# Ledicia/Molecular-Dynamics-Simulation---Lennard-Jones-monoatomic-fluid

Hardware: AMD Instinct MI355X
Metric: md_steps_per_sec_n262144_fp64 (higher is better)
Workload: dtype f64

## Files before the change

molecular-dynamics-simulation---lennard-jones-monoatomic-fluid_amd/csrc/ljmd_common.cpp:

```cpp
#include "ljmd_common.h"
#include "ljmd_internal.h"

#include <algorithm>
#include <cstdio>
#include <cstring>
#include <limits>

namespace ljmdh {

using namespace ljmdk;

thread_local std::string g_last_error = "";

int failv(std::string *handle_err, int code, const char *fmt, va_list ap)
{
    char buf[512];
    vsnprintf(buf, sizeof buf, fmt, ap);
    g_last_error = buf;
    if (handle_err) *handle_err = buf;
    return code;
}

int check_sim_params(const char *who, int n, double box_length, double dt, double rc)
{
// ... 51 lines not shown
        if (v && *v) return std::atoi(v);
        return std::nullopt;
    };
    Knobs k;
    k.sort = flag("LJMD_SORT", k.sort);
    k.force_generic = flag("LJMD_FORCE_GENERIC", k.force_generic);
    k.force_collectives = flag("LJMD_FORCE_COLLECTIVES", k.force_collectives);
    k.fuse = flag("LJMD_FUSE", k.fuse);
    k.fuse_tail = flag("LJMD_FUSE_TAIL", k.fuse_tail);
    k.fuse_defer_record = flag("LJMD_FUSE_DEFER_RECORD", k.fuse_defer_record);
    k.xcd_remap = std::max(0, env_int("LJMD_N3_XCD_REMAP", k.xcd_remap));
    k.inject_failure_at_step = env_int("LJMD_INJECT_FAILURE_AT_STEP", k.inject_failure_at_step);
    k.exchange_alltoall = is("LJMD_FORCE_EXCHANGE", "alltoall");
    k.resort_every = opt_int("LJMD_RESORT_EVERY");
    k.n3_row_tiles = env_int("LJMD_N3_ROW_TILES", k.n3_row_tiles);
    k.n3_wg_waves = env_int("LJMD_N3_WG_WAVES", k.n3_wg_waves);
    k.slab_budget_gb = std::max(1, env_int("LJMD_SLAB_BUDGET_GB", k.slab_budget_gb));
    k.n3_both_ties = flag("LJMD_N3_BOTH_TIES", k.n3_both_ties);
    k.n3_min_n = env_int("LJMD_N3_MIN_N", k.n3_min_n);
    k.n3 = flag("LJMD_N3", k.n3);
    k.n3_target_waves = opt_int("LJMD_N3_TARGET_WAVES");
    k.n3_clusters = flag("LJMD_N3_CLUSTERS", k.n3_clusters);
    k.n3_pertile = flag("LJMD_N3_PERTILE", k.n3_pertile);
    k.fp32_far_stream = flag("LJMD_FP32_FAR_STREAM", k.fp32_far_stream);
    k.fp32_vfar = flag("LJMD_FP32_VFAR", k.fp32_vfar);
    {
        const char *rs = std::getenv("LJMD_FP32_SPLIT");
        if (rs && *rs) k.fp32_split = std::max(0.0, std::atof(rs));
    }
    k.overlap_exchange = flag("LJMD_OVERLAP_EXCHANGE", k.overlap_exchange);
    k.migrate_blocks = is("LJMD_MIGRATE_DEAL", "blocks");
    {
        const char *xm = std::getenv("LJMD_MULTI_EXCHANGE");
        k.multi_exchange = xm ? xm : "";
    }
    k.multi_migrate_every = std::max(0, env_int("LJMD_MULTI_MIGRATE_EVERY", k.multi_migrate_every));
    k.multi_threads = flag("LJMD_MULTI_THREADS", k.multi_threads);
    k.batch_group_streams = !is("LJMD_BATCH_GROUP_STREAMS", "0");
    return k;
}

void scalars_from_sums(double s12, double s6, double kx, double ky, double kz, double te, double td, double tdd,
                       double *epot, double *ekin, double *d_epot, double *dd_epot)
{
    if (epot) *epot = 4.0 * (s12 - s6) + te;
    if (d_epot) *d_epot = 24.0 * (-2.0 * s12 + s6) + td;
// ... 67 lines not shown
```

molecular-dynamics-simulation---lennard-jones-monoatomic-fluid_amd/csrc/ljmd_common.h:

```cpp
#ifndef LJMD_COMMON_H
#define LJMD_COMMON_H

#include "ljmd.h"

#include <hip/hip_runtime.h>

#include <cstdarg>
#include <cstddef>
#include <cstdint>
#include <cstdlib>
#include <optional>
#include <string>

namespace ljmdh {

extern thread_local std::string g_last_error;

constexpr double kPi = 3.1415926535897932384626433832795;

int failv(std::string *handle_err, int code, const char *fmt, va_list ap);

inline int fail(std::nullptr_t, int code, const char *fmt, ...)
{
    va_list ap;
// ... 49 lines not shown
void scalars_from_exact_sums(const uint64_t (&ordered)[5][3], double te, double td, double tdd, bool have_e, bool have_k,
                             double *epot, double *ekin, double *d_epot, double *dd_epot);

struct Knobs {
    bool sort = true;
    bool force_generic = false;
    bool force_collectives = false;
    bool fuse = true;
    bool fuse_tail = true;
    bool fuse_defer_record = true;
    int xcd_remap = 4;
    int inject_failure_at_step = -1;
    bool exchange_alltoall = false;
    std::optional<int> resort_every;
    int n3_row_tiles = 0;
    int n3_wg_waves = 0;
    int slab_budget_gb = 64;
    bool n3_both_ties = true;
    int n3_min_n = 4096;
    bool n3 = true;
    std::optional<int> n3_target_waves;
    bool n3_clusters = true;
    bool n3_pertile = true;
    bool fp32_far_stream = true;
    bool fp32_vfar = true;
    double fp32_split = 5.0;
    bool overlap_exchange = true;
    bool migrate_blocks = false;
    std::string multi_exchange;
    int multi_migrate_every = 2000;
    bool multi_threads = true;
    bool batch_group_streams = true;
};
Knobs read_knobs();

}
#endif
```

molecular-dynamics-simulation---lennard-jones-monoatomic-fluid_amd/csrc/ljmd_engine.cpp:

```cpp
#include "ljmd_engine.h"

namespace ljmdh {

bool fast_path_ok(const ljmd_t *h) { return h->plan.rc_allows_fast && h->positions_compact && !h->knobs.force_generic; }

double *wg_part_now(ljmd_t *h) { return h->d_wg_part + (h->plan.fuse_tail ? (size_t)h->fold_parity * h->wg_part_stride : 0); }

PairArgs pair_args(ljmd_t *h, bool fast)
{
    PairArgs a;
    a.pos = h->d_pos;
    a.slab = h->d_slab;
    a.wg_part = wg_part_now(h);
    a.mask = h->d_mask;
    a.bbox = h->d_bbox;
    a.inline_mask = (fast && h->plan.fuse_tail && !h->plan.use_n3) ? 1 : 0;
    a.rc2_skin = h->rc2 * (1.0 + 1e-10);
    a.n = h->n;
    a.S = h->plan.S;
    a.P = h->plan.P;
    a.G = h->G;
    a.rank = h->rank;
    a.TB = h->plan.TB;
    a.T = h->plan.T;
// ... 36 lines not shown
    a.pos = h->d_pos_tc;
    a.mask = h->d_mask;
    a.bbox = h->d_bbox;
    a.desc = h->d_desc;
    a.desc2 = h->d_desc2;
    a.slab_i = h->d_slab;
    a.slab_j = h->d_slab_j;
    a.flag_j = h->d_flag_j;
    a.wg_part = wg_part_now(h);
    a.S = h->plan.S;
    a.P = h->plan.P;
    a.G = h->G;
    a.rank = h->rank;
    a.TB = h->plan.TB;
    a.T = h->plan.T;
    a.W = h->plan.W;
    a.NG = h->plan.NG;
    a.NGo = h->plan.NGo;
    a.Dmax = h->plan.Dmax;
    a.CS = h->plan.CS;
    a.by_group = h->plan.j_by_group;
    a.dchunk = h->plan.dchunk;
    a.uchunk = h->plan.uchunk;
    a.xcd_remap = 0;
    a.inline_class = (h->plan.fuse_tail && h->plan.rt <= 2 && h->plan.wg_waves == 1) ? 1 : 0;
    a.both_ties = h->plan.both_ties ? 1 : 0;
    a.rc2_skin = h->rc2 * (1.0 + 1e-10);
    a.energy = h->want_energy ? 1 : 0;
    a.RT = h->plan.rt;
    a.L = h->L;
    a.invL = h->invL;
    a.rc2 = h->rc2;
    return a;
}

IntegrateArgs integrate_args(ljmd_t *h)
{
    IntegrateArgs a;
    a.r = own_block(h);
    a.ru = h->d_ru;
    a.v = h->d_v;
    a.a = h->d_a;
    a.fsum = needs_force_exchange(h) ? h->d_frecv : h->d_fpart;
    a.bbox = nullptr;
    a.pos_tc = nullptr;
    a.RT = std::max(1, h->plan.rt);
// ... 6 lines not shown
    a.dt = h->dt;
    a.dt_half = h->dt_half;
    a.dt_sq_half = h->dt_sq_half;
    return a;
}

ReduceArgs reduce_args(ljmd_t *h, int nslab, bool n3)
{
    ReduceArgs a;
    a.slab = h->d_slab;
    a.slab_j = n3 ? h->d_slab_j : nullptr;
    a.flag_j = n3 ? h->d_flag_j : nullptr;
    a.slab_j2 = (n3 && h->mode == LJMD_PRECISION_FP32_FORCE) ? reinterpret_cast<const float *>(h->d_slab_j2) : nullptr;
    a.flag_j2 = (n3 && h->mode == LJMD_PRECISION_FP32_FORCE) ? h->d_flag_j2 : nullptr;
    a.fpart = h->d_fpart;
    a.nslab = nslab;
    a.P = h->plan.P;
    a.G = h->G;
    a.rank = h->rank;
    a.TB = h->plan.TB;
    a.CS = h->plan.CS;
    a.CS2 = h->plan.CS2;
    a.RT = h->plan.rt;
    return a;
}

FinalizeArgs finalize_args(ljmd_t *h, int n_wg, bool with_ke, double pair_scale)
{
    FinalizeArgs a;
    a.pair_scale = pair_scale;
    a.wg_part = wg_part_now(h);
    a.ke_part = h->d_ke_part;
    a.ke_tile = nullptr;
    a.ring = h->d_ring;
    a.ring_pos = h->d_ring_pos;
    a.n_wg = n_wg;
    a.n_ke = with_ke ? h->plan.n_ke : 0;
    a.ring_cap = kRingCap;
    return a;
}

EventSet *next_events(ljmd_t *h)
{
    if (!h->profiling || h->ev_used >= (size_t)kMaxProfiledLaunches) return nullptr;
    if (h->ev_used == h->ev_pool.size()) {
        EventSet q;
// ... 84 lines not shown
            LJMD_HIP(h, launch_tile_mask(ga, h->stream));
        }
        h->boxes_valid = false;
        if (q) LJMD_HIP(h, hipEventRecord(q->e[2], h->stream));
        FixedArgs fa;
        fa.pos = h->d_pos;
        fa.mask = h->d_mask;
        fa.fslab = h->d_fslab;
        fa.fflag = h->d_fflag;
        fa.walk_all = fast ? 0 : 1;
        fa.S = h->plan.S; fa.P = h->plan.P; fa.G = h->G; fa.rank = h->rank; fa.TB = h->plan.TB; fa.T = h->plan.T; fa.W = h->plan.W;
        fa.chunk = h->plan.chunk_t;
        fa.energy = h->want_energy ? 1 : 0;
        fa.L = h->L; fa.invL = h->invL; fa.rc2 = h->rc2;
        LJMD_HIP(h, launch_pair_fixed(fa, dim3(h->plan.TB / kWavesPerBlock, h->plan.nslab_t), h->stream));
        if (q) LJMD_HIP(h, hipEventRecord(q->e[3], h->stream));
        h->pending_energy = h->want_energy;
        h->reduce_deferred = false;
        h->forces_pending = true;
        return LJMD_OK;
    }
    int nslab, n_wg;
    bool n3 = false;
    if (fast) {
        GeometryArgs ga = geometry_args(h);
        if (!h->plan.use_n3) ga.mask_far = nullptr;
        if (!h->boxes_valid) LJMD_HIP(h, launch_tile_boxes(ga, h->stream));
        h->boxes_valid = false;
        if (h->plan.fuse_tail)
            ;
        else if (h->plan.use_n3)
            LJMD_HIP(h, launch_tile_class(ga, h->invL, h->rc2, h->plan.S, h->plan.NGo, h->d_desc,
                                          h->mode == LJMD_PRECISION_FP32_FORCE ? h->d_desc_far : nullptr, h->d_desc2, h->stream));
        else
            LJMD_HIP(h, launch_tile_mask(ga, h->stream));
        if (q) LJMD_HIP(h, hipEventRecord(q->e[2], h->stream));
        if (h->plan.use_n3) {
            const dim3 grid((h->plan.NGo + h->plan.wg_waves - 1) / h->plan.wg_waves, h->plan.nslab_n);
            N3Args na = n3_args(h);
            na.xcd_remap = (h->knobs.xcd_remap > 0 && (int)grid.x >= kXcdMinGroups && grid.x % (8 * h->knobs.xcd_remap) == 0) ? h->knobs.xcd_remap : 0;
            const bool far_beside = h->mode == LJMD_PRECISION_FP32_FORCE && h->far_stream != nullptr;
            if (far_beside) {
                LJMD_HIP(h, hipEventRecord(h->ev_far_go, h->stream));
                LJMD_HIP(h, hipStreamWaitEvent(h->far_stream, h->ev_far_go, 0));
            } else {
                LJMD_HIP(h, launch_pair_n3(na, grid, h->plan.wg_waves, h->stream));
            }
            nslab = h->plan.nslab_n;
            n_wg = grid.x * grid.y * h->plan.wg_waves;
            n3 = true;
            if (h->mode == LJMD_PRECISION_FP32_FORCE) {
                const dim3 fgrid(h->plan.NGo, h->plan.nslab_n);
                N3Args fa = n3_args(h);
                fa.mask = h->d_mask_far;
                fa.slab_i = h->d_slab + (size_t)h->plan.nslab_n * 3 * h->plan.P;
                fa.slab_j = h->d_slab_j2;
                fa.flag_j = h->d_flag_j2;
                fa.desc = h->d_desc_far;
                fa.CS = h->plan.CS2;
                fa.by_group = h->G > 1 ? 1 : 0;
                fa.xcd_remap = (h->knobs.xcd_remap > 0 && (int)fgrid.x >= kXcdMinGroups && fgrid.x % (8 * h->knobs.xcd_remap) == 0) ? h->knobs.xcd_remap : 0;
                fa.wg_part = h->d_wg_part + 2 * (size_t)n_wg;
                LJMD_HIP(h, launch_pair_n3_f32(fa, fgrid, far_beside ? h->far_stream : h->stream));
                if (far_beside) {
                    LJMD_HIP(h, hipEventRecord(h->ev_far_done, h->far_stream));
// ... 4 lines not shown
                n_wg += fgrid.x * fgrid.y;
            }
        } else {
            const dim3 grid(h->plan.TB / kWavesPerBlock, h->plan.nslab_t);
            LJMD_HIP(h, launch_pair_tiles(pair_args(h, true), grid, h->stream));
            nslab = h->plan.nslab_t;
            n_wg = grid.x * grid.y;
        }
    } else {
        if (h->plan.use_n3 && h->G > 1)
            return fail(h, LJMD_ERR_STATE,
                        "multi-rank Newton-3 run needs wrapped positions and rc <= (1-1e-9) L/2 (set LJMD_N3=0)");
        if (q) LJMD_HIP(h, hipEventRecord(q->e[2], h->stream));
        const dim3 grid(h->plan.P / kBlock, h->plan.nslab_g);
        LJMD_HIP(h, launch_pair_rows_generic(pair_args(h, false), grid, h->stream));
        nslab = h->plan.nslab_g;
        n_wg = grid.x * grid.y;
    }
    if (q) LJMD_HIP(h, hipEventRecord(q->e[3], h->stream));
    h->reduce_deferred = fast && h->plan.fuse_tail && h->kick_hint >= 0 && n_wg <= kDirectFoldMax && !needs_force_exchange(h);
    if (h->reduce_deferred) {
        h->deferred_nslab = nslab;
        h->deferred_n3 = n3;
    } else {
        LJMD_HIP(h, launch_reduce_forces(reduce_args(h, nslab, n3), needs_force_exchange(h), h->stream));
    }
    h->forces_pending = true;
    h->pending_n_wg = n_wg;
    h->pending_scale = n3 ? 1.0 : 0.5;
    return LJMD_OK;
}

int enqueue_kick(ljmd_t *h, bool kick, EventSet *q)
{
    if (reproducible(h)) {
        FixedTailArgs ta;
        ta.fslab = h->d_fslab;
        ta.fflag = h->d_fflag;
        ta.nslab = h->plan.nslab_t;
        ta.P = h->plan.P;
        ta.TB = h->plan.TB;
        ta.a = h->d_a;
        ta.v = h->d_v;
        ta.dt_half = h->dt_half;
        ta.blk = h->d_fblk;
        LJMD_HIP(h, launch_fixed_tail(ta, kick, h->pending_energy, false, h->stream));
// ... 196 lines not shown
```

molecular-dynamics-simulation---lennard-jones-monoatomic-fluid_amd/csrc/ljmd_engine.h:

```cpp
#ifndef LJMD_ENGINE_H
#define LJMD_ENGINE_H

#include "ljmd_common.h"

#include <rccl/rccl.h>

#include <algorithm>
#include <cmath>
#include <cstdio>
#include <cstring>
#include <limits>
#include <mutex>
#include <vector>

#include "ljmd_internal.h"
#include "ljmd_rdf.h"
#include "ljmd_tcf.h"

using namespace ljmdk;

namespace ljmdh {

constexpr unsigned kRingCap = 4096;
constexpr int kTargetWorkgroups = 2048;
constexpr int kXcdMinGroups = 256;
constexpr int kMixedMinN = 16384;
constexpr long kN3ItemsFor4 = 6000;
constexpr long kN3ItemsFor2 = 1000;
constexpr long kN3LargeItems = 131072;
constexpr int kN3MidTargetItems = 32768;
constexpr int kBothTiesMaxGroups = 128;
constexpr int kFuseTailMaxRowTiles = 2;
constexpr int kFuseTailMaxN = 20000;
constexpr int kMaxProfiledLaunches = 4096;
constexpr int kEventsPerLaunch = 9;

struct EventSet {
    hipEvent_t e[kEventsPerLaunch];
    bool has_pos_x = false, has_force_x = false;
};

struct LaunchPlan {
    int S = 0, P = 0;
    int TB = 0, T = 0, W = 0;
    bool rc_allows_fast = false;
    bool sort_enabled = true;
    int resort_every = 20;
    std::vector<int> kd_level_nseg;
    std::vector<size_t> kd_level_off;
    std::vector<int> kd_offsets;
    int nslab_g = 1, chunk_g = 0;
    int nslab_t = 1, chunk_t = 0;
    bool use_n3 = false;
    int wg_waves = 1;
    bool both_ties = false;
    int uchunk = 0;
    int CS = 0, CS2 = 0, j_by_group = 0;
    int NG = 0, NGo = 0, Dmax = 0, nslab_n = 1, dchunk = 0;
    int rt = kRowTiles;
    bool fuse_tail = false;
    int nslab_max = 1, n_wg_max = 0;
    int n_ke = 0;
};

int plan_engine(const SimParams &sim, int n, int n_ranks, int precision_mode, const Knobs &k, LaunchPlan *out);

}

struct ljmd_multi;

using namespace ljmdh;

struct ljmd : ljmdh::SimParams {
    ljmd_multi *multi = nullptr;
    bool poisoned = false;
    int inject_failure_at = -1;
    int n = 0, rank = 0, G = 1, device = 0, mode = 0;
    ljmdh::Knobs knobs;
    ljmdh::LaunchPlan plan;
    bool tail_on = true;
    bool positions_compact = false;
    bool have_state = false, have_accel = false;
    int steps_since_sort = 0;
// ... 28 lines not shown
    unsigned *d_ring_pos = nullptr;
    double *d_bbox = nullptr;
    uint64_t *d_mask = nullptr;
    double *d_pos_tc = nullptr;
    unsigned *d_desc = nullptr;
    unsigned *d_desc_far = nullptr;
    float *d_desc2 = nullptr;
    int *d_idx = nullptr, *d_idx2 = nullptr, *d_perm = nullptr, *d_perm2 = nullptr;
    double *d_tmp3 = nullptr;
    void *d_cub = nullptr;
    size_t cub_bytes = 0;
    std::vector<int> kd_axis;
    int *d_kd_offsets = nullptr;
    unsigned long long *d_kd_keys = nullptr, *d_kd_keys2 = nullptr;

    unsigned ring_consumed = 0;
    unsigned ring_issued = 0;
    bool fold_pending = false;
    ljmdk::FinalizeArgs pending_fold{};
    int fold_parity = 0;
    size_t wg_part_stride = 0;
    double *d_slab_j = nullptr;
    unsigned char *d_flag_j = nullptr;
    uint64_t *d_mask_far = nullptr;
    double *d_slab_j2 = nullptr;
    unsigned char *d_flag_j2 = nullptr;
    double *d_fpart = nullptr, *d_frecv = nullptr;
    double *d_fall = nullptr;
    bool forces_pending = false;
    bool external_force_exchange = false;
    int pending_n_wg = 0;
    double pending_scale = 0.5;

    double *h_stage = nullptr;
    double *h_ring = nullptr;
    std::vector<int> h_perm;
    bool perm_dirty = false;

    hipStream_t far_stream = nullptr;
    hipEvent_t ev_far_go = nullptr, ev_far_done = nullptr;
    hipStream_t copy_stream = nullptr;
    hipEvent_t ev_snap_ready = nullptr, ev_snap_done = nullptr;
    double *d_snap = nullptr, *h_snap = nullptr;
    int *d_snap_perm = nullptr, *h_snap_perm = nullptr;
    bool snap_in_flight = false;
    bool snap_ready = false;
// ... 72 lines not shown
```

molecular-dynamics-simulation---lennard-jones-monoatomic-fluid_amd/csrc/ljmd_internal.h:

```cpp
#ifndef LJMD_INTERNAL_H
#define LJMD_INTERNAL_H

#include <hip/hip_runtime.h>
#include <stdint.h>

namespace ljmdk {

constexpr int kBlock = 256;
constexpr int kWavesPerBlock = kBlock / 64;
constexpr int kTile = 64;
#ifndef LJMD_ROW_TILES
#define LJMD_ROW_TILES 4
#endif
constexpr int kRowTiles = LJMD_ROW_TILES;
constexpr unsigned kAllRows = (1u << kRowTiles) - 1u;
constexpr int kSlotAlign = (kRowTiles * 64 > 256) ? kRowTiles * 64 : 256;
constexpr int kPartialStride = 8;
constexpr int kFoldBlocks = 128;
constexpr int kDirectFoldMax = 20480;
constexpr int kBoxStride = 8;

struct PairArgs {
    const double *pos;
    double *slab;
// ... 9 lines not shown
    int rank;
    int TB;
    int T;
    int W;
    int chunk;
    double L, invL, rc2;
};

struct N3Args {
    const double *pos;
    const uint64_t *mask;
    const double *bbox;
    const unsigned *desc;
    const float *desc2;
    double *slab_i;
    double *slab_j;
    unsigned char *flag_j;
    double *wg_part;
    int S, P, G, rank, TB, T, W;
    int NG, NGo, Dmax;
    int CS, by_group;
    int RT;
    int dchunk;
    int uchunk;
    int energy;
    int xcd_remap;
    int inline_class;
    int both_ties;
    double L, invL, rc2;
    double rc2_skin;
};

struct IntegrateArgs {
    double *r;
    double *ru, *v, *a;
    const double *fsum;
    double *ke_part;
    int rows;
    int P;
    double L, invL, dt, dt_half, dt_sq_half;
    double *bbox;
    double *pos_tc;
    int RT;
    unsigned *ticket;
};

struct ReduceArgs {
    const double *slab;
    const double *slab_j;
    const unsigned char *flag_j;
    const float *slab_j2;
    const unsigned char *flag_j2;
    double *fpart;
    int nslab, P, G, rank, TB;
    int CS, CS2;
    int RT;
};

struct FinalizeArgs {
    const double *wg_part;
    const double *ke_part;
    const double *ke_tile;
    double *ring;
    unsigned *ring_pos;
    int n_wg, n_ke;
    unsigned ring_cap;
    double pair_scale;
};

struct GeometryArgs {
    const double *pos;
    double *bbox;
    double *pos_tc;
    uint64_t *mask;
    uint64_t *mask_far;
    int P, G, rank, TB, T, W;
    int RT;
    double L, invL, rc2_skin;
    double rsplit2;
// ... 97 lines not shown
    return neg ? -r : r;
}

struct RdfArgs {
    const double *x, *y, *z;
    unsigned long long *hist;
    int n, nbins, chunk;
    double L, rmax, dr;
    double invL, inv_dr;
};

struct TimeOriginArgs {
    const double *x, *y, *z;
    double *term;
    int n_snap, n, max_lag, origin_stride;
};

hipError_t launch_pair_rows_generic(const PairArgs &a, dim3 grid, hipStream_t s);
hipError_t launch_pair_tiles(const PairArgs &a, dim3 grid, hipStream_t s);
hipError_t launch_pair_n3(const N3Args &a, dim3 grid, int wg_waves, hipStream_t s);
hipError_t launch_pair_n3_f32(const N3Args &a, dim3 grid, hipStream_t s);
hipError_t launch_drift_kick(const IntegrateArgs &a, int phase , hipStream_t s);
hipError_t launch_reduce_forces(const ReduceArgs &a, bool all_blocks, hipStream_t s);
hipError_t launch_kick(const IntegrateArgs &a, bool kick, hipStream_t s);
hipError_t launch_kick_finalize(const IntegrateArgs &a, const FinalizeArgs &f, bool kick, hipStream_t s);
hipError_t launch_kinetic_fused(const IntegrateArgs &a, hipStream_t s);
hipError_t launch_sum_blocks(const double *blocks, double *out, int G, int len, hipStream_t s);
hipError_t launch_finalize(const FinalizeArgs &a, double *fold_scratch , hipStream_t s);
hipError_t launch_tile_tail(const ReduceArgs &ra, const IntegrateArgs &a, const FinalizeArgs &f, const FinalizeArgs &prev, bool kick,
                            bool drift, hipStream_t s);
hipError_t launch_pair_fixed(const FixedArgs &a, dim3 grid, hipStream_t s);
hipError_t launch_fixed_tail(const FixedTailArgs &a, bool kick, bool energy, bool ke_only, hipStream_t s);
hipError_t launch_fixed_fold(const FixedFoldArgs &a, hipStream_t s);
hipError_t launch_rdf_histogram(const RdfArgs &a, dim3 grid, hipStream_t s);
hipError_t launch_time_origin(const TimeOriginArgs &a, bool vacf, int n_origins, hipStream_t s);
hipError_t launch_tile_boxes(const GeometryArgs &a, hipStream_t s);
hipError_t launch_tile_mask(const GeometryArgs &a, hipStream_t s);
hipError_t launch_tile_class(const GeometryArgs &a, double invL, double rc2, int S, int NGo, unsigned *desc,
                             unsigned *desc_far, float *desc2 , hipStream_t s);

size_t kd_temp_bytes(int count);
hipError_t launch_iota(int *idx, int P, hipStream_t s);
hipError_t kd_level(void *temp, size_t temp_bytes, const double *coord_axis, double L, unsigned long long *keys,
                    unsigned long long *keys_out, int *idx, int *idx_out, int S, int nseg, const int *seg_offsets,
                    hipStream_t s);
constexpr int kMigrateRows = 10;
// ... 184 lines not shown
```

molecular-dynamics-simulation---lennard-jones-monoatomic-fluid_amd/csrc/ljmd_kernels.hip:

```cpp
#include <hip/hip_runtime.h>
#include <stdint.h>

#include "ljmd_internal.h"

namespace ljmdk {

__device__ __forceinline__ double wave_min(double v)
{
#pragma unroll
    for (int off = 32; off > 0; off >>= 1) v = fmin(v, __shfl_down(v, off, 64));
    return v;
}

__device__ __forceinline__ double wave_max(double v)
{
#pragma unroll
    for (int off = 32; off > 0; off >>= 1) v = fmax(v, __shfl_down(v, off, 64));
    return v;
}

__global__ __launch_bounds__(kBlock) void pair_rows_generic_kernel(PairArgs a)
{
    __shared__ double red[2 * kWavesPerBlock];
    const int row = blockIdx.x * kBlock + threadIdx.x;
// ... 795 lines not shown
            }
        }
    }
    desc_out = mb | cls;
    if (desc_far) desc_far[(size_t)Al * a.T + c] = mb_far | cls | ((unsigned)(vfar && full && mb_far != 0) << 28);
    return true;
}

template <int MIN_WAVES, int RT, int W, bool ENERGY>
__global__ __launch_bounds__(kTile * W, MIN_WAVES) void pair_n3_kernel(N3Args a)
{
    __shared__ double parked_all[W][3 * kLdsAxis];
    __shared__ double comb[W > 1 ? 2 : 1][W][3][W > 1 ? kTile : 1];
    __shared__ int comb_on[2][W];
    const int lane = threadIdx.x & 63;
    const int wv = W == 1 ? 0 : __builtin_amdgcn_readfirstlane((int)(threadIdx.x >> 6));
    unsigned bx = blockIdx.x, by = blockIdx.y;
    if (a.xcd_remap) {
        const unsigned id = blockIdx.y * gridDim.x + blockIdx.x, per = gridDim.x >> 3, C = (unsigned)a.xcd_remap;
        const unsigned xcd = id & 7u, slot = id >> 3, s = slot % per;
        by = slot / per;
        bx = ((s / C) * 8u + xcd) * C + s % C;
    }
#ifdef LJMD_WAVE_TRACE
    const unsigned long long tr0 = trace_now();
    unsigned long long tr1 = tr0;
    unsigned tr_heavy = 0;
#endif
    const int Al = (int)bx * W + wv;
    const bool active = Al < a.NGo;
    const int A = a.rank * a.NGo + Al;
    const int A0 = a.rank * a.NGo + (int)bx * W;
    const size_t P = a.P;
    const double *own = a.pos + (size_t)a.rank * 3 * P;

    double xi[RT], yi[RT], zi[RT];
    double ax[RT], ay[RT], az[RT];
    double s12 = 0.0, s6 = 0.0;
#pragma unroll
    for (int k = 0; k < RT; ++k) {
        const size_t slot = (size_t)(active ? RT * Al + k : 0) * kTile + lane;
        xi[k] = own[slot];
        yi[k] = own[P + slot];
        zi[k] = own[2 * P + slot];
        ax[k] = ay[k] = az[k] = 0.0;
    }
// ... 513 lines not shown
                    }
                }
                f = fn;
            }
        };
        add_blocks(a.slab_j, a.flag_j, a.CS);
        if (a.slab_j2) add_blocks(a.slab_j2, a.flag_j2, a.CS2);
    }
    part[q][0][lane] = s[0];
    part[q][1][lane] = s[1];
    part[q][2][lane] = s[2];
    __syncthreads();
    if (q == 0) {
#pragma unroll
        for (int ax = 0; ax < 3; ++ax) {
            double t = part[0][ax][lane];
#pragma unroll
            for (int w = 1; w < kWavesPerBlock; ++w) t += part[w][ax][lane];
            a.fpart[(size_t)(gridDim.y == 1 ? 0 : g) * 3 * a.P + (size_t)ax * a.P + i] = t;
        }
    }
}

template <bool KICK>
__global__ __launch_bounds__(kBlock) void kick_kernel(IntegrateArgs a)
{
    __shared__ double red[3 * kWavesPerBlock];
    const int i = blockIdx.x * kBlock + threadIdx.x;
    double k2[3] = {0.0, 0.0, 0.0};
    if (i < a.rows) {
#pragma unroll
        for (int ax = 0; ax < 3; ++ax) {
            const size_t o = (size_t)ax * a.P + i;
            const double acc = 24.0 * a.fsum[o];
            a.a[o] = acc;
            if constexpr (KICK) {
                const double v1 = a.v[o] + acc * a.dt_half;
                a.v[o] = v1;
                k2[ax] = v1 * v1;
            }
        }
    }
    if constexpr (KICK) {
        block_sum<3>(k2, red);
        if (threadIdx.x == 0) {
            double *w = a.ke_part + 3 * (size_t)blockIdx.x;
// ... 529 lines not shown
{
    const dim3 grid((a.rows + kBlock - 1) / kBlock);
    if (phase == 1)
        hipLaunchKernelGGL(drift_kick_kernel<1>, grid, dim3(kBlock), 0, s, a);
    else if (phase == 2)
        hipLaunchKernelGGL(drift_kick_kernel<2>, grid, dim3(kBlock), 0, s, a);
    else if (a.bbox)
        hipLaunchKernelGGL((drift_kick_kernel<0, true>), grid, dim3(kBlock), 0, s, a);
    else
        hipLaunchKernelGGL(drift_kick_kernel<0>, grid, dim3(kBlock), 0, s, a);
    return hipGetLastError();
}

hipError_t launch_reduce_forces(const ReduceArgs &a, bool all_blocks, hipStream_t s)
{
    const dim3 grid(a.P / kTile, all_blocks ? a.G : 1);
    if (a.slab_j)
        hipLaunchKernelGGL(reduce_forces_kernel<true>, grid, dim3(kBlock), 0, s, a);
    else
        hipLaunchKernelGGL(reduce_forces_kernel<false>, grid, dim3(kBlock), 0, s, a);
    return hipGetLastError();
}

hipError_t launch_kick(const IntegrateArgs &a, bool kick, hipStream_t s)
{
    const dim3 grid((a.rows + kBlock - 1) / kBlock);
    if (kick)
        hipLaunchKernelGGL(kick_kernel<true>, grid, dim3(kBlock), 0, s, a);
    else
        hipLaunchKernelGGL(kick_kernel<false>, grid, dim3(kBlock), 0, s, a);
    return hipGetLastError();
}

hipError_t launch_kick_finalize(const IntegrateArgs &a, const FinalizeArgs &f, bool kick, hipStream_t s)
{
    const dim3 grid((a.rows + kBlock - 1) / kBlock);
    if (kick)
        hipLaunchKernelGGL(kick_finalize_kernel<true>, grid, dim3(kBlock), 0, s, a, f);
    else
        hipLaunchKernelGGL(kick_finalize_kernel<false>, grid, dim3(kBlock), 0, s, a, f);
    return hipGetLastError();
}

__global__ __launch_bounds__(kBlock) void sum_blocks_kernel(const double *blocks, double *out, int G, int len)
{
    const int i = blockIdx.x * kBlock + threadIdx.x;
// ... 90 lines not shown
```

molecular-dynamics-simulation---lennard-jones-monoatomic-fluid_amd/csrc/ljmd_plan.cpp:

```cpp
#include "ljmd_engine.h"

namespace ljmdh {

int plan_engine(const SimParams &sim, int n, int n_ranks, int precision_mode, const Knobs &k, LaunchPlan *out)
{
    LaunchPlan p;
    p.S = n / n_ranks;
    p.P = ((p.S + kSlotAlign - 1) / kSlotAlign) * kSlotAlign;
    p.TB = p.P / kTile;
    p.T = n_ranks * p.TB;
    p.W = (p.T + 63) / 64;
    p.rc_allows_fast = sim.rc <= (1.0 - 1e-9) * 0.5 * sim.L;
    p.sort_enabled = k.sort && n >= 1024;
    p.resort_every = std::max(1, k.resort_every.value_or(n >= 1000000 ? 5 : n >= 131072 ? 10 : n > 40000 ? 20
                                                              : n > kFuseTailMaxN ? 50 : 200));
    {
        const int tiles = (p.S + kTile - 1) / kTile;
        std::vector<int> bounds = {0, tiles};
        while (true) {
            bool any = false;
            for (size_t j = 0; j + 1 < bounds.size(); ++j) any = any || (bounds[j + 1] - bounds[j] > 1);
            if (!any) break;
            p.kd_level_off.push_back(p.kd_offsets.size());
            p.kd_level_nseg.push_back((int)bounds.size() - 1);
            for (int b : bounds) p.kd_offsets.push_back(std::min(b * kTile, p.S));
// ... 46 lines not shown
        p.CS = p.j_by_group ? (p.NGo + wg - 1) / wg : (p.Dmax + wg - 1) / wg + 1;
        p.CS2 = n_ranks > 1 ? p.NGo : p.Dmax + 1;
        p.use_n3 = k.n3 && n >= k.n3_min_n && (n_ranks == 1 || p.rc_allows_fast) &&
                   precision_mode != LJMD_PRECISION_FP64_REPRODUCIBLE;
        const int n_off = p.Dmax + p.wg_waves;
        const int n_units = n_off * rt;
        const bool plenty = (long)p.NGo * n_off >= kN3LargeItems || n_ranks > 1;
        const int target_waves = std::max(1, k.n3_target_waves.value_or(plenty ? 131072 : kN3MidTargetItems));
        const int ns_wanted = (target_waves + p.NGo - 1) / p.NGo;
        int ns = std::max(1, std::min(ns_wanted, n_off));
        const bool small_single = n_ranks == 1 && n <= kFuseTailMaxN && rt <= kFuseTailMaxRowTiles;
        const int ns_cap = small_single ? std::max(1, kDirectFoldMax / std::max(1, p.NGo)) : n_units;
        ns = std::min(ns, ns_cap);
        p.dchunk = (n_off + ns - 1) / ns;
        p.uchunk = p.dchunk * rt;
        if (!mixed_mode && ns_wanted > n_off) {
            const int nsu = std::max(1, std::min(std::min(ns_wanted, ns_cap), n_units));
            p.uchunk = (n_units + nsu - 1) / nsu;
        }
        p.nslab_n = (n_units + p.uchunk - 1) / p.uchunk;
    }
    p.fuse_tail = k.fuse && k.fuse_tail && n_ranks == 1 && n <= kFuseTailMaxN && p.rc_allows_fast &&
                  precision_mode == LJMD_PRECISION_FP64 && (!p.use_n3 || (p.rt <= kFuseTailMaxRowTiles && p.wg_waves == 1));
    const bool mixed = precision_mode == LJMD_PRECISION_FP32_FORCE;
    if (mixed && (!p.use_n3 || n < kMixedMinN))
        return fail(nullptr, LJMD_ERR_INVALID_ARG,
                    "ljmd_create: LJMD_PRECISION_FP32_FORCE needs the Newton-3 path and n >= %d", kMixedMinN);
    p.nslab_max = std::max(std::max(p.nslab_g, p.nslab_t), p.use_n3 ? p.nslab_n * (mixed ? 2 : 1) : 1);
    p.n_wg_max = std::max(row_blocks * std::max(p.nslab_g, p.nslab_t),
                          (p.NGo + 4) * p.nslab_n * (mixed ? 2 : 1));
    p.n_ke = row_blocks;
    *out = std::move(p);
    return LJMD_OK;
}

}
```

molecular-dynamics-simulation---lennard-jones-monoatomic-fluid_amd/csrc/ljmd_storage.cpp:

```cpp
#include "ljmd_engine.h"

namespace ljmdh {

int allocate_engine(ljmd_t *h)
{
    const bool mixed = h->mode == LJMD_PRECISION_FP32_FORCE;
    const std::vector<int> &kd = h->plan.kd_offsets;
    LJMD_HIP(h, hipSetDevice(h->device));
    LJMD_HIP(h, hipStreamCreateWithFlags(&h->stream, hipStreamNonBlocking));
    const size_t P3 = 3 * (size_t)h->plan.P * sizeof(double);
    LJMD_HIP(h, hipMalloc(&h->d_pos, P3 * h->G));
    LJMD_HIP(h, hipMalloc(&h->d_ru, P3));
    LJMD_HIP(h, hipMalloc(&h->d_v, P3));
    LJMD_HIP(h, hipMalloc(&h->d_a, P3));
    LJMD_HIP(h, hipMalloc(&h->d_tmp3, P3));
    LJMD_HIP(h, hipMalloc(&h->d_slab, P3 * h->plan.nslab_max));
    h->wg_part_stride = 2 * (size_t)h->plan.n_wg_max;
    LJMD_HIP(h, hipMalloc(&h->d_wg_part, (h->plan.fuse_tail ? 2 : 1) * h->wg_part_stride * sizeof(double)));
    if (h->plan.use_n3) {
        const size_t n_blk = (size_t)h->plan.T * h->plan.CS;
        LJMD_HIP(h, hipMalloc(&h->d_slab_j, n_blk * 3 * kTile * sizeof(double)));
        LJMD_HIP(h, hipMalloc(&h->d_flag_j, n_blk));
        LJMD_HIP(h, hipMemsetAsync(h->d_flag_j, 0, n_blk, h->stream));
        LJMD_HIP(h, hipMalloc(&h->d_desc, (size_t)h->plan.NGo * h->plan.T * sizeof(unsigned)));
        if (h->plan.rt == kRowTiles && h->plan.wg_waves == 1 && h->knobs.n3_clusters)
            LJMD_HIP(h, hipMalloc(&h->d_desc2, (size_t)h->plan.NGo * h->plan.T * 8 * sizeof(float)));
        LJMD_HIP(h, hipMalloc(&h->d_pos_tc, P3 * h->G));
    }
    if (mixed && h->knobs.fp32_far_stream) {
        LJMD_HIP(h, hipStreamCreateWithFlags(&h->far_stream, hipStreamNonBlocking));
        LJMD_HIP(h, hipEventCreateWithFlags(&h->ev_far_go, hipEventDisableTiming));
        LJMD_HIP(h, hipEventCreateWithFlags(&h->ev_far_done, hipEventDisableTiming));
    }
    if (mixed) {
        LJMD_HIP(h, hipMalloc(&h->d_mask_far, (size_t)h->plan.TB * h->plan.W * sizeof(uint64_t)));
        LJMD_HIP(h, hipMalloc(&h->d_desc_far, (size_t)h->plan.NGo * h->plan.T * sizeof(unsigned)));
        const size_t n_blk2 = (size_t)h->plan.T * h->plan.CS2;
        LJMD_HIP(h, hipMalloc(&h->d_slab_j2, n_blk2 * 3 * kTile * sizeof(float)));
        LJMD_HIP(h, hipMalloc(&h->d_flag_j2, n_blk2));
        LJMD_HIP(h, hipMemsetAsync(h->d_flag_j2, 0, n_blk2, h->stream));
    }
    LJMD_HIP(h, hipMalloc(&h->d_fpart, P3 * (needs_force_exchange(h) ? h->G : 1)));
    if (needs_force_exchange(h)) LJMD_HIP(h, hipMalloc(&h->d_frecv, P3));
    if (needs_force_exchange(h) && h->knobs.exchange_alltoall) LJMD_HIP(h, hipMalloc(&h->d_fall, P3 * h->G));
    LJMD_HIP(h, hipMalloc(&h->d_ke_part, 3 * (size_t)h->plan.n_ke * sizeof(double)));
    LJMD_HIP(h, hipMalloc(&h->d_fold, 2 * (size_t)kFoldBlocks * sizeof(double)));
    LJMD_HIP(h, hipMalloc(&h->d_ticket, sizeof(unsigned)));
    LJMD_HIP(h, hipMemsetAsync(h->d_ticket, 0, sizeof(unsigned), h->stream));
    if (h->plan.fuse_tail) {
        LJMD_HIP(h, hipMalloc(&h->d_ke_tile, 2 * 3 * (size_t)h->plan.T * sizeof(double)));
// ... 28 lines not shown
    LJMD_HIP(h, hipMemsetAsync(h->d_a, 0, P3, h->stream));
    LJMD_HIP(h, hipMemsetAsync(h->d_ke_part, 0, 3 * (size_t)h->plan.n_ke * sizeof(double), h->stream));
    LJMD_HIP(h, hipHostMalloc(&h->h_stage, P3 * std::max(h->G, 4), hipHostMallocDefault));
    LJMD_HIP(h, hipHostMalloc(&h->h_ring, (size_t)kRingCap * h->rec_stride * sizeof(double),
                              hipHostMallocDefault));
    LJMD_HIP(h, hipStreamSynchronize(h->stream));
    return LJMD_OK;
}

void release(ljmd_t *h)
{
    if (!h) return;
    if (h->device >= 0) (void)hipSetDevice(h->device);
    if (h->stream) (void)hipStreamSynchronize(h->stream);
    ljmdr::rdf_release(&h->rdf, h->stream);
    ljmdt::tcf_release(&h->tcf, h->stream);
    if (h->comm_stream) (void)hipStreamSynchronize(h->comm_stream);
    if (h->comm) (void)ncclCommDestroy(h->comm);
    if (h->comm_stream) (void)hipStreamDestroy(h->comm_stream);
    if (h->far_stream) {
        (void)hipStreamSynchronize(h->far_stream);
        (void)hipStreamDestroy(h->far_stream);
    }
    if (h->ev_far_go) (void)hipEventDestroy(h->ev_far_go);
    if (h->ev_far_done) (void)hipEventDestroy(h->ev_far_done);
    if (h->ev_pos_ready) (void)hipEventDestroy(h->ev_pos_ready);
    if (h->ev_gather_done) (void)hipEventDestroy(h->ev_gather_done);
    for (auto &q : h->ev_pool)
        for (auto &e : q.e) (void)hipEventDestroy(e);
    void *dev[] = {h->d_pos, h->d_ru, h->d_v, h->d_a, h->d_slab, h->d_wg_part, h->d_ke_part, h->d_ring,
                   h->d_ring_pos, h->d_bbox, h->d_mask, h->d_idx, h->d_idx2,
                   h->d_perm, h->d_perm2, h->d_tmp3, h->d_cub, h->d_slab_j, h->d_flag_j, h->d_fpart, h->d_frecv, h->d_fall,
                   h->d_kd_offsets, h->d_kd_keys, h->d_kd_keys2, h->d_mask_far, h->d_slab_j2, h->d_flag_j2, h->d_fold, h->d_ticket,
                   h->d_desc, h->d_desc_far, h->d_desc2, h->d_ke_tile, h->d_pos_tc, h->d_gid0, h->d_mig, h->d_mig_idx, h->d_mig_idx2, h->d_mig_keys,
                   h->d_mig_keys2, h->d_mig_offsets, h->d_mig_cub, h->d_fslab, h->d_fflag, h->d_fblk, h->d_frec};
    for (void *p : dev) (void)hipFree(p);
    if (h->h_stage) (void)hipHostFree(h->h_stage);
    if (h->h_ring) (void)hipHostFree(h->h_ring);
    if (h->copy_stream) {
        (void)hipStreamSynchronize(h->copy_stream);
        (void)hipStreamDestroy(h->copy_stream);
    }
    if (h->ev_snap_ready) (void)hipEventDestroy(h->ev_snap_ready);
    if (h->ev_snap_done) (void)hipEventDestroy(h->ev_snap_done);
    if (h->d_snap) (void)hipFree(h->d_snap);
    if (h->d_snap_perm) (void)hipFree(h->d_snap_perm);
    if (h->h_snap) (void)hipHostFree(h->h_snap);
    if (h->h_snap_perm) (void)hipHostFree(h->h_snap_perm);
    if (h->stream) (void)hipStreamDestroy(h->stream);
    delete h;
}

int download_state(ljmd_t *h, double *const dsts[12], unsigned n_records)
{
    const size_t P = h->plan.P;
    const double *srcs[4] = {own_block(h), h->d_ru, h->d_v, h->d_a};
    bool want[4];
// ... 63 lines not shown
```

Before: 54.94.

## Split N3 pair grid and overlap first-phase force reduction with remaining tiles

Splits the Newton-3 pair kernel grid along y into a main-stream part and a low-priority side-stream part. A two-phase reduction kernel sums the first part's slabs and j-blocks into a partial buffer while the side-stream tiles still compute, then a second phase finishes the remaining slabs and writes the forces. The aim is to hide most of the reduction latency behind the pair-kernel tail. The cost is an extra partial buffer, event sync, and the risk of contention or an uneven split. It is enabled by default for fp64 single-rank runs with n >= 131072.

```diff
diff --git a/molecular-dynamics-simulation---lennard-jones-monoatomic-fluid_amd/csrc/ljmd_common.cpp b/molecular-dynamics-simulation---lennard-jones-monoatomic-fluid_amd/csrc/ljmd_common.cpp
--- a/molecular-dynamics-simulation---lennard-jones-monoatomic-fluid_amd/csrc/ljmd_common.cpp
+++ b/molecular-dynamics-simulation---lennard-jones-monoatomic-fluid_amd/csrc/ljmd_common.cpp
@@ -97,6 +97,8 @@
     k.n3_target_waves = opt_int("LJMD_N3_TARGET_WAVES");
     k.n3_clusters = flag("LJMD_N3_CLUSTERS", k.n3_clusters);
     k.n3_pertile = flag("LJMD_N3_PERTILE", k.n3_pertile);
+    k.reduce_split = opt_int("LJMD_REDUCE_SPLIT");
+    if (k.reduce_split) k.reduce_split = std::max(0, *k.reduce_split);
     k.fp32_far_stream = flag("LJMD_FP32_FAR_STREAM", k.fp32_far_stream);
     k.fp32_vfar = flag("LJMD_FP32_VFAR", k.fp32_vfar);
     {
diff --git a/molecular-dynamics-simulation---lennard-jones-monoatomic-fluid_amd/csrc/ljmd_common.h b/molecular-dynamics-simulation---lennard-jones-monoatomic-fluid_amd/csrc/ljmd_common.h
--- a/molecular-dynamics-simulation---lennard-jones-monoatomic-fluid_amd/csrc/ljmd_common.h
+++ b/molecular-dynamics-simulation---lennard-jones-monoatomic-fluid_amd/csrc/ljmd_common.h
@@ -95,6 +95,7 @@
     std::optional<int> n3_target_waves;
     bool n3_clusters = true;
     bool n3_pertile = true;
+    std::optional<int> reduce_split;
     bool fp32_far_stream = true;
     bool fp32_vfar = true;
     double fp32_split = 5.0;
diff --git a/molecular-dynamics-simulation---lennard-jones-monoatomic-fluid_amd/csrc/ljmd_engine.cpp b/molecular-dynamics-simulation---lennard-jones-monoatomic-fluid_amd/csrc/ljmd_engine.cpp
--- a/molecular-dynamics-simulation---lennard-jones-monoatomic-fluid_amd/csrc/ljmd_engine.cpp
+++ b/molecular-dynamics-simulation---lennard-jones-monoatomic-fluid_amd/csrc/ljmd_engine.cpp
@@ -82,6 +82,7 @@
     a.by_group = h->plan.j_by_group;
     a.dchunk = h->plan.dchunk;
     a.uchunk = h->plan.uchunk;
+    a.by0 = 0;
     a.xcd_remap = 0;
     a.inline_class = (h->plan.fuse_tail && h->plan.rt <= 2 && h->plan.wg_waves == 1) ? 1 : 0;
     a.both_ties = h->plan.both_ties ? 1 : 0;
@@ -134,6 +135,9 @@
     a.CS = h->plan.CS;
     a.CS2 = h->plan.CS2;
     a.RT = h->plan.rt;
+    a.partial = h->d_red_part;
+    a.c_split = h->plan.split_s1;
+    a.j_split = h->plan.split_j1;
     return a;
 }
 
@@ -264,6 +268,7 @@
     }
     int nslab, n_wg;
     bool n3 = false;
+    bool split = false;
     if (fast) {
         GeometryArgs ga = geometry_args(h);
         if (!h->plan.use_n3) ga.mask_far = nullptr;
@@ -282,7 +287,19 @@
             N3Args na = n3_args(h);
             na.xcd_remap = (h->knobs.xcd_remap > 0 && (int)grid.x >= kXcdMinGroups && grid.x % (8 * h->knobs.xcd_remap) == 0) ? h->knobs.xcd_remap : 0;
             const bool far_beside = h->mode == LJMD_PRECISION_FP32_FORCE && h->far_stream != nullptr;
-            if (far_beside) {
+            split = h->plan.split_s1 > 0 && h->side_stream != nullptr;
+            if (split) {
+                const int s1 = h->plan.split_s1;
+                LJMD_HIP(h, hipEventRecord(h->ev_side_go, h->stream));
+                LJMD_HIP(h, hipStreamWaitEvent(h->side_stream, h->ev_side_go, 0));
+                LJMD_HIP(h, launch_pair_n3(na, dim3(grid.x, s1), h->plan.wg_waves, h->stream));
+                N3Args nb = na;
+                nb.by0 = s1;
+                LJMD_HIP(h, launch_pair_n3(nb, dim3(grid.x, grid.y - s1), h->plan.wg_waves, h->side_stream));
+                LJMD_HIP(h, launch_reduce_forces_split(reduce_args(h, h->plan.nslab_n, true), 1, h->stream));
+                LJMD_HIP(h, hipEventRecord(h->ev_side_done, h->side_stream));
+                LJMD_HIP(h, hipStreamWaitEvent(h->stream, h->ev_side_done, 0));
+            } else if (far_beside) {
                 LJMD_HIP(h, hipEventRecord(h->ev_far_go, h->stream));
                 LJMD_HIP(h, hipStreamWaitEvent(h->far_stream, h->ev_far_go, 0));
             } else {
@@ -333,6 +350,8 @@
     if (h->reduce_deferred) {
         h->deferred_nslab = nslab;
         h->deferred_n3 = n3;
+    } else if (split) {
+        LJMD_HIP(h, launch_reduce_forces_split(reduce_args(h, nslab, n3), 2, h->stream));
     } else {
         LJMD_HIP(h, launch_reduce_forces(reduce_args(h, nslab, n3), needs_force_exchange(h), h->stream));
     }
diff --git a/molecular-dynamics-simulation---lennard-jones-monoatomic-fluid_amd/csrc/ljmd_engine.h b/molecular-dynamics-simulation---lennard-jones-monoatomic-fluid_amd/csrc/ljmd_engine.h
--- a/molecular-dynamics-simulation---lennard-jones-monoatomic-fluid_amd/csrc/ljmd_engine.h
+++ b/molecular-dynamics-simulation---lennard-jones-monoatomic-fluid_amd/csrc/ljmd_engine.h
@@ -32,6 +32,8 @@
 constexpr int kBothTiesMaxGroups = 128;
 constexpr int kFuseTailMaxRowTiles = 2;
 constexpr int kFuseTailMaxN = 20000;
+constexpr int kReduceSplitMinN = 131072;
+constexpr int kReduceSplitShare = 8;
 constexpr int kMaxProfiledLaunches = 4096;
 constexpr int kEventsPerLaunch = 9;
 
@@ -59,6 +61,7 @@
     int NG = 0, NGo = 0, Dmax = 0, nslab_n = 1, dchunk = 0;
     int rt = kRowTiles;
     bool fuse_tail = false;
+    int split_s1 = 0, split_j1 = 0;
     int nslab_max = 1, n_wg_max = 0;
     int n_ke = 0;
 };
@@ -133,6 +136,9 @@
     size_t wg_part_stride = 0;
     double *d_slab_j = nullptr;
     unsigned char *d_flag_j = nullptr;
+    double *d_red_part = nullptr;
+    hipStream_t side_stream = nullptr;
+    hipEvent_t ev_side_go = nullptr, ev_side_done = nullptr;
     uint64_t *d_mask_far = nullptr;
     double *d_slab_j2 = nullptr;
     unsigned char *d_flag_j2 = nullptr;
diff --git a/molecular-dynamics-simulation---lennard-jones-monoatomic-fluid_amd/csrc/ljmd_internal.h b/molecular-dynamics-simulation---lennard-jones-monoatomic-fluid_amd/csrc/ljmd_internal.h
--- a/molecular-dynamics-simulation---lennard-jones-monoatomic-fluid_amd/csrc/ljmd_internal.h
+++ b/molecular-dynamics-simulation---lennard-jones-monoatomic-fluid_amd/csrc/ljmd_internal.h
@@ -55,6 +55,7 @@
     int CS, by_group;
     int RT;
     int dchunk;
+    int by0;
     int uchunk;
     int energy;
     int xcd_remap;
@@ -88,6 +89,8 @@
     int nslab, P, G, rank, TB;
     int CS, CS2;
     int RT;
+    double *partial;
+    int c_split, j_split;
 };
 
 struct FinalizeArgs {
@@ -231,6 +234,7 @@
 hipError_t launch_pair_n3_f32(const N3Args &a, dim3 grid, hipStream_t s);
 hipError_t launch_drift_kick(const IntegrateArgs &a, int phase , hipStream_t s);
 hipError_t launch_reduce_forces(const ReduceArgs &a, bool all_blocks, hipStream_t s);
+hipError_t launch_reduce_forces_split(const ReduceArgs &a, int phase , hipStream_t s);
 hipError_t launch_kick(const IntegrateArgs &a, bool kick, hipStream_t s);
 hipError_t launch_kick_finalize(const IntegrateArgs &a, const FinalizeArgs &f, bool kick, hipStream_t s);
 hipError_t launch_kinetic_fused(const IntegrateArgs &a, hipStream_t s);
diff --git a/molecular-dynamics-simulation---lennard-jones-monoatomic-fluid_amd/csrc/ljmd_kernels.hip b/molecular-dynamics-simulation---lennard-jones-monoatomic-fluid_amd/csrc/ljmd_kernels.hip
--- a/molecular-dynamics-simulation---lennard-jones-monoatomic-fluid_amd/csrc/ljmd_kernels.hip
+++ b/molecular-dynamics-simulation---lennard-jones-monoatomic-fluid_amd/csrc/ljmd_kernels.hip
@@ -841,6 +841,7 @@
         by = slot / per;
         bx = ((s / C) * 8u + xcd) * C + s % C;
     }
+    by += (unsigned)a.by0;
 #ifdef LJMD_WAVE_TRACE
     const unsigned long long tr0 = trace_now();
     unsigned long long tr1 = tr0;
@@ -1400,6 +1401,82 @@
     }
 }
 
+template <int PHASE>
+__global__ __launch_bounds__(kBlock) void reduce_forces_split_kernel(ReduceArgs a)
+{
+    __shared__ double part[kWavesPerBlock][3][kTile];
+    const int lane = threadIdx.x & 63, q = threadIdx.x >> 6;
+    const int i = blockIdx.x * kTile + lane;
+    double *mine = a.partial + ((size_t)blockIdx.x * kWavesPerBlock + q) * (3 * kTile) + lane;
+    double s[3] = {0.0, 0.0, 0.0};
+    if constexpr (PHASE == 2) {
+        s[0] = mine[0];
+        s[1] = mine[kTile];
+        s[2] = mine[2 * kTile];
+    }
+    const int c_lo = PHASE == 1 ? 0 : a.c_split, c_hi = PHASE == 1 ? a.c_split : a.nslab;
+    for (int c = c_lo + ((q - c_lo) & (kWavesPerBlock - 1)); c < c_hi; c += kWavesPerBlock) {
+        const double *sl = a.slab + (size_t)c * 3 * a.P + i;
+        s[0] += sl[0];
+        s[1] += sl[a.P];
+        s[2] += sl[2 * (size_t)a.P];
+    }
+    {
+        constexpr int U = 4;
+        const int j_lo = PHASE == 1 ? 0 : a.j_split, j_hi = PHASE == 1 ? a.j_split : a.CS;
+        const int qs = __builtin_amdgcn_readfirstlane(q);
+        const size_t base = (size_t)blockIdx.x * a.CS;
+        const int j_first = j_lo & ~(kTile - 1);
+        unsigned f = j_first + lane < j_hi ? a.flag_j[base + j_first + lane] : 0u;
+        for (int j0 = j_first; j0 < j_hi; j0 += kTile) {
+            unsigned long long m = __ballot(f != 0u && j0 + lane >= j_lo) & (0x1111111111111111ull << qs);
+            const int jn = j0 + kTile + lane;
+            const unsigned fn = jn < j_hi ? a.flag_j[base + jn] : 0u;
+            while (m) {
+                double v[U][3];
+#pragma unroll
+                for (int u = 0; u < U; ++u) {
+                    v[u][0] = v[u][1] = v[u][2] = 0.0;
+                    if (m) {
+                        const int j = j0 + __builtin_ctzll(m);
+                        m &= m - 1;
+                        const double *b = a.slab_j + (base + j) * (3 * kTile) + lane;
+                        v[u][0] = b[0];
+                        v[u][1] = b[kTile];
+                        v[u][2] = b[2 * kTile];
+                    }
+                }
+#pragma unroll
+                for (int u = 0; u < U; ++u) {
+                    s[0] += v[u][0];
+                    s[1] += v[u][1];
+                    s[2] += v[u][2];
+                }
+            }
+            f = fn;
+        }
+    }
+    if constexpr (PHASE == 1) {
+        mine[0] = s[0];
+        mine[kTile] = s[1];
+        mine[2 * kTile] = s[2];
+    } else {
+        part[q][0][lane] = s[0];
+        part[q][1][lane] = s[1];
+        part[q][2][lane] = s[2];
+        __syncthreads();
+        if (q == 0) {
+#pragma unroll
+            for (int ax = 0; ax < 3; ++ax) {
+                double t = part[0][ax][lane];
+#pragma unroll
+                for (int w = 1; w < kWavesPerBlock; ++w) t += part[w][ax][lane];
+                a.fpart[(size_t)ax * a.P + i] = t;
+            }
+        }
+    }
+}
+
 template <bool KICK>
 __global__ __launch_bounds__(kBlock) void kick_kernel(IntegrateArgs a)
 {
@@ -1975,6 +2052,16 @@
     return hipGetLastError();
 }
 
+hipError_t launch_reduce_forces_split(const ReduceArgs &a, int phase, hipStream_t s)
+{
+    const dim3 grid(a.P / kTile);
+    if (phase == 1)
+        hipLaunchKernelGGL(reduce_forces_split_kernel<1>, grid, dim3(kBlock), 0, s, a);
+    else
+        hipLaunchKernelGGL(reduce_forces_split_kernel<2>, grid, dim3(kBlock), 0, s, a);
+    return hipGetLastError();
+}
+
 hipError_t launch_kick(const IntegrateArgs &a, bool kick, hipStream_t s)
 {
     const dim3 grid((a.rows + kBlock - 1) / kBlock);
diff --git a/molecular-dynamics-simulation---lennard-jones-monoatomic-fluid_amd/csrc/ljmd_plan.cpp b/molecular-dynamics-simulation---lennard-jones-monoatomic-fluid_amd/csrc/ljmd_plan.cpp
--- a/molecular-dynamics-simulation---lennard-jones-monoatomic-fluid_amd/csrc/ljmd_plan.cpp
+++ b/molecular-dynamics-simulation---lennard-jones-monoatomic-fluid_amd/csrc/ljmd_plan.cpp
@@ -1,6 +1,15 @@
 #include "ljmd_engine.h"
 
 namespace ljmdh {
+
+namespace {
+int rt_align(int uchunk, int rt)
+{
+    int m = 1;
+    while ((m * uchunk) % rt != 0) ++m;
+    return m;
+}
+}
 
 int plan_engine(const SimParams &sim, int n, int n_ranks, int precision_mode, const Knobs &k, LaunchPlan *out)
 {
@@ -93,6 +102,17 @@
     }
     p.fuse_tail = k.fuse && k.fuse_tail && n_ranks == 1 && n <= kFuseTailMaxN && p.rc_allows_fast &&
                   precision_mode == LJMD_PRECISION_FP64 && (!p.use_n3 || (p.rt <= kFuseTailMaxRowTiles && p.wg_waves == 1));
+    if (n_ranks == 1 && precision_mode == LJMD_PRECISION_FP64 && p.use_n3 && p.rc_allows_fast && !p.fuse_tail &&
+        p.rt == kRowTiles && p.wg_waves == 1 && !p.j_by_group && !k.force_collectives) {
+        const int S = p.nslab_n;
+        const int m = rt_align(p.uchunk, p.rt);
+        const int deferred = k.reduce_split.value_or(n >= kReduceSplitMinN ? (S + kReduceSplitShare - 1) / kReduceSplitShare : 0);
+        if (deferred >= 1 && m < S) {
+            const int s1 = std::max(m, (std::max(0, S - deferred) / m) * m);
+            p.split_s1 = s1;
+            p.split_j1 = s1 * p.uchunk / p.rt;
+        }
+    }
     const bool mixed = precision_mode == LJMD_PRECISION_FP32_FORCE;
     if (mixed && (!p.use_n3 || n < kMixedMinN))
         return fail(nullptr, LJMD_ERR_INVALID_ARG,
diff --git a/molecular-dynamics-simulation---lennard-jones-monoatomic-fluid_amd/csrc/ljmd_storage.cpp b/molecular-dynamics-simulation---lennard-jones-monoatomic-fluid_amd/csrc/ljmd_storage.cpp
--- a/molecular-dynamics-simulation---lennard-jones-monoatomic-fluid_amd/csrc/ljmd_storage.cpp
+++ b/molecular-dynamics-simulation---lennard-jones-monoatomic-fluid_amd/csrc/ljmd_storage.cpp
@@ -26,6 +26,14 @@
         if (h->plan.rt == kRowTiles && h->plan.wg_waves == 1 && h->knobs.n3_clusters)
             LJMD_HIP(h, hipMalloc(&h->d_desc2, (size_t)h->plan.NGo * h->plan.T * 8 * sizeof(float)));
         LJMD_HIP(h, hipMalloc(&h->d_pos_tc, P3 * h->G));
+    }
+    if (h->plan.split_s1 > 0) {
+        LJMD_HIP(h, hipMalloc(&h->d_red_part, (size_t)h->plan.TB * kWavesPerBlock * 3 * kTile * sizeof(double)));
+        int least = 0, greatest = 0;
+        LJMD_HIP(h, hipDeviceGetStreamPriorityRange(&least, &greatest));
+        LJMD_HIP(h, hipStreamCreateWithPriority(&h->side_stream, hipStreamNonBlocking, least));
+        LJMD_HIP(h, hipEventCreateWithFlags(&h->ev_side_go, hipEventDisableTiming));
+        LJMD_HIP(h, hipEventCreateWithFlags(&h->ev_side_done, hipEventDisableTiming));
     }
     if (mixed && h->knobs.fp32_far_stream) {
         LJMD_HIP(h, hipStreamCreateWithFlags(&h->far_stream, hipStreamNonBlocking));
@@ -100,6 +108,12 @@
         (void)hipStreamSynchronize(h->far_stream);
         (void)hipStreamDestroy(h->far_stream);
     }
+    if (h->side_stream) {
+        (void)hipStreamSynchronize(h->side_stream);
+        (void)hipStreamDestroy(h->side_stream);
+    }
+    if (h->ev_side_go) (void)hipEventDestroy(h->ev_side_go);
+    if (h->ev_side_done) (void)hipEventDestroy(h->ev_side_done);
     if (h->ev_far_go) (void)hipEventDestroy(h->ev_far_go);
     if (h->ev_far_done) (void)hipEventDestroy(h->ev_far_done);
     if (h->ev_pos_ready) (void)hipEventDestroy(h->ev_pos_ready);
@@ -110,7 +124,7 @@
                    h->d_ring_pos, h->d_bbox, h->d_mask, h->d_idx, h->d_idx2,
                    h->d_perm, h->d_perm2, h->d_tmp3, h->d_cub, h->d_slab_j, h->d_flag_j, h->d_fpart, h->d_frecv, h->d_fall,
                    h->d_kd_offsets, h->d_kd_keys, h->d_kd_keys2, h->d_mask_far, h->d_slab_j2, h->d_flag_j2, h->d_fold, h->d_ticket,
-                   h->d_desc, h->d_desc_far, h->d_desc2, h->d_ke_tile, h->d_pos_tc, h->d_gid0, h->d_mig, h->d_mig_idx, h->d_mig_idx2, h->d_mig_keys,
+                   h->d_desc, h->d_desc_far, h->d_desc2, h->d_red_part, h->d_ke_tile, h->d_pos_tc, h->d_gid0, h->d_mig, h->d_mig_idx, h->d_mig_idx2, h->d_mig_keys,
                    h->d_mig_keys2, h->d_mig_offsets, h->d_mig_cub, h->d_fslab, h->d_fflag, h->d_fblk, h->d_frec};
     for (void *p : dev) (void)hipFree(p);
     if (h->h_stage) (void)hipHostFree(h->h_stage);
```

Measured after the change: 57.15, median of 6. 4.0% higher.
